# pdh930105/ARCQuant

Measured on AMD Instinct MI355X. Metric: ARC-NVFP4 GEMM TFLOP/s (M=4096, N=KQ=4096, KE=64), higher is better.
Workload: dtype f16

## Files before the change

arcquant_amd/agemm.py:

```python
from __future__ import annotations

import functools

import torch

from . import _lib
from ._lib import VARIANT_G16, VARIANT_G32, OUT_BF16, OUT_F32, ArcqError

_raw_stream = getattr(torch._C, "_cuda_getCurrentRawStream", None)


def _stream(t: torch.Tensor) -> int:
    if _raw_stream is not None:
        return _raw_stream(t.get_device())
    return torch.cuda.current_stream(t.device).cuda_stream


class _on:
    __slots__ = ("ctx",)

    def __init__(self, device):
        idx = device.index
        self.ctx = None if idx is None or idx == torch.cuda.current_device() else torch.cuda.device(device)

# ... 47 lines not shown
        return float(scale_host), scale, scale.data_ptr()
    return float(scale_host) * float(scale), None, None


_OUT_CODES = {torch.bfloat16: OUT_BF16, torch.float32: OUT_F32}


def _out(out, M, N, out_dtype, like, who):
    code = _OUT_CODES.get(out_dtype)
    if code is None:
        raise RuntimeError(f"agemm.{who}: out_dtype must be bfloat16 or float32")
    if out is None:
        return torch.empty((M, N), dtype=out_dtype, device=like.device), code
    _need(out, out_dtype, "out", 2)
    if out.shape != (M, N):
        raise RuntimeError(f"agemm.{who}: out has the wrong shape, expected ({M}, {N})")
    return out, code


def _same_device(who: str, A: torch.Tensor, *ts):
    idx = A.get_device()
    if idx < 0:
        raise RuntimeError(f"agemm.{who}: the operands must live on the GPU (there is no CPU path)")
    for t in ts:
        if t is not None and t.get_device() != idx:
            raise RuntimeError(f"agemm.{who}: every operand must live on the GPU of the first one ({A.device}), got {t.device}")


def _debug_set_tile_overlap_tail(mode: int) -> None:
    fn = _lib.lib().arcq_debug_set_tile_overlap_tail
    fn.restype, fn.argtypes = None, [_lib._i32]
    fn(int(mode))
    rw_route.cache_clear()


@functools.lru_cache(maxsize=None)
def variant_for_kq(KQ: int) -> int:
    return int(_lib.lib().arcq_variant_for_kq(int(KQ)))


@functools.lru_cache(maxsize=None)
def sf_buffer_bytes(rows: int, K: int) -> int:
    return int(_lib.lib().arcq_sf_alloc_bytes(int(rows), int(K)))


@functools.lru_cache(maxsize=None)
def _sf_used(rows: int, K: int) -> int:
    return int(_lib.lib().arcq_sf_used_bytes(int(rows), int(K)))


@functools.lru_cache(maxsize=None)
def _repacked_bytes(N: int, K: int):
    L = _lib.lib()
    return int(L.arcq_repacked_w_bytes(N, K)), int(L.arcq_repacked_sf_bytes(N, K))


def _need_repacked(RW, RSF, SFA, M, N, K, who, n_mult=1):
    _need(RW, torch.uint8, "RW", 1)
    _need(RSF, torch.uint8, "RSF", 1)
    if K % 64 or N % n_mult or (RW.numel(), RSF.numel()) != _repacked_bytes(N, K):
        raise RuntimeError(f"Value error in {who}: RW / RSF do not belong to a [{N}, {K}] weight" + (f", or N % {n_mult} != 0" if n_mult > 1 else ""))
    if SFA is not None and SFA.numel() < _sf_used(M, K):
        raise RuntimeError(f"Value error in {who}: SFA smaller than the swizzled layout of A")


def _quantize(fn_name: str, X: torch.Tensor, reorder_index: torch.Tensor, KE: int, variant):
# ... 475 lines not shown
```

arcquant_amd/csrc/arcq_internal.hpp:

```cpp
#pragma once
#include <hip/hip_runtime.h>
#include <stdint.h>
#include <stdlib.h>

#include "../../include/arcq.h"

namespace arcq {

int fail(int code, const char* fmt, ...) __attribute__((format(printf, 2, 3)));

inline int env_int(const char* name, int dflt) {
  const char* e = getenv(name);
  return e ? atoi(e) : dflt;
}

constexpr int kMaxDevices = 64;
struct LdsOptIn {
  int granted[kMaxDevices];
};
int ensure_dynamic_lds(const void* kernel, LdsOptIn& cache, int bytes, const char* who);

struct LdsBytes {
  int launch, optin;
  LdsBytes(int bytes) : launch(bytes), optin(bytes) {}
// ... 91 lines not shown
  const uint16_t* X;
  const uint16_t* Wn;
  float eps;
  const int16_t* idx;
  const uint32_t* in_slots;
  int n_in_slots;
  float* scale_out;
  const uint8_t* RW;
  const uint8_t* RSF;
  void* D;
  uint32_t* out_slots;
  const int16_t* act_scatter;
  int M, N, KQ, KE, variant;
  float alpha_host;
  const float* alpha_dev;
  const uint16_t* bias;
  const uint16_t* residual;
  int out_dtype;
};
int gemm_fused_supported(int kind, int64_t M, int64_t N, int64_t KQ, int64_t KE);
int gemm_fused(const FusedArgs& f, hipStream_t stream);
int64_t gemm_skinny_workspace_bytes(int64_t M, int64_t N, int64_t K);
int64_t gemm_tile_workspace_bytes(int64_t M, int64_t N, int64_t K);
int64_t gemm_tile_silu_slots(int64_t M, int64_t N, int64_t K);
int64_t gemm_decode_silu_slots(int64_t M, int64_t N, int64_t K);
int gemm_splitk_finish(const GemmArgs& a, int splitk, hipStream_t stream);
int gemm_skinny(const GemmArgs& a, hipStream_t stream);
int64_t gemm_decode_workspace_bytes(int64_t M, int64_t N, int64_t K);
int gemm_decode(const GemmArgs& a, hipStream_t stream);
int gemm_tile(const GemmArgs& a, hipStream_t stream);
int gemm_tile_repacked(const GemmArgs& a, hipStream_t stream);
int tile_overlap_tail_mode();
inline bool tile_overlap_tail_forced(int64_t M, int64_t N) { return tile_overlap_tail_mode() == 2 && M % 256 == 0 && N % 256 == 0; }
int gemm_regtile_cfg(int64_t M, int64_t N, int64_t K, int epilogue);
int gemm_regtile(const GemmArgs& a, int cfg, hipStream_t stream);
int gemm_regtile_fits(int64_t M, int64_t N, int64_t K, int b_layout);

struct KvWriteArgs {
  void* kv_data;
  void* kv_param;
  const int32_t *kv_indptr, *kv_indices, *last_page_offset;
  const void *k, *v, *k_param, *v_param;
  const int32_t* seqlen_indptr;
  int64_t ntok, B, L, layer, N, P;
  int format, dtype;
  bool quantize;
};
int kv_write(const KvWriteArgs& a, hipStream_t stream);
struct KvDecodeArgs {
  void* o;
  const void *q, *kv_data, *kv_param;
  const int32_t *kv_indptr, *kv_indices, *last_page_offset;
  int64_t B, Nq, L, layer, N, P, nnz;
  int format, dtype;
  void* workspace;
};
int kv_decode_splits(int64_t B, int64_t Nq, int64_t N, int64_t nnz, int64_t P);
int kv_decode(const KvDecodeArgs& a, hipStream_t stream);
struct KvStepArgs {
  const void *k, *v;
  int64_t q_stride, kv_stride;
  void* state;
};
int64_t kv_decode_chunks(int64_t Nq, int64_t N);
int kv_decode_step(const KvDecodeArgs& a, const KvStepArgs& st, hipStream_t stream);

// ... 13 lines not shown
```

arcquant_amd/csrc/gemm_tile.hip:

```cpp
#include <hip/hip_runtime.h>
#include <stdint.h>
#include <stdlib.h>

#include <type_traits>

#include "arcq_internal.hpp"
#include "gemm_common.hpp"
#include "gemm_tile_common.hpp"

namespace arcq {

#ifdef ARCQ_STREAM_STAMPS
#ifndef ARCQ_TILE_OT_UNIT
static unsigned long long* g_tile_stamps = nullptr;
#ifndef ARCQ_TILE_REPACKED_UNIT
extern "C" void arcq_debug_set_tile_stamps(void* p) { g_tile_stamps = reinterpret_cast<unsigned long long*>(p); }
#endif
#endif
#define ARCQ_TILE_STAMP(k)                                                                                     \
  do {                                                                                                         \
    if (p.stamps && tid == 0) {                                                                                \
      unsigned long long t0_, t1_;                                                                             \
      asm volatile("s_memtime %0\n\ts_memrealtime %1\n\ts_waitcnt lgkmcnt(0)" : "=s"(t0_), "=s"(t1_)::"memory"); \
      p.stamps[(size_t)blockIdx.x * (2 * kTileStamps) + 2 * (k)] = t0_;                                        \
      p.stamps[(size_t)blockIdx.x * (2 * kTileStamps) + 2 * (k) + 1] = t1_;                                    \
    }                                                                                                          \
  } while (0)
#else
#define ARCQ_TILE_STAMP(k) do { } while (0)
#endif

#ifndef ARCQ_TILE_WIDE_STORES
#define ARCQ_TILE_WIDE_STORES 1
#endif

#ifndef ARCQ_TILE_BARRIER_AT_STEP_END
#define ARCQ_TILE_BARRIER_AT_STEP_END 0
#endif
#ifndef ARCQ_TILE_ROT
#define ARCQ_TILE_ROT 1
#endif

#ifndef ARCQ_TILE_OT_UNIT
template <int BM, int BN, int WAVES_M, int WAVES_N, bool kMfma32, int kEpi, bool kStagger, bool kPipe, int kBLayout = kBRef>
__global__ __launch_bounds__(WAVES_M* WAVES_N * 64) void gemm_tile_kernel(TileParams p) {
  constexpr bool kOverlapTail = false;
  [[maybe_unused]] constexpr int kEpiOps = 0;
#else
template <int BM, int BN, int WAVES_M, int WAVES_N, int kEpi, int kBLayout, int kEpiOps>
__global__ __launch_bounds__(WAVES_M* WAVES_N * 64) void gemm_tile_ot_kernel(TileParams p) {
  static_assert(kEpiOps >= 0 && kEpiOps < (kEpi == kEpiSiluMul ? 2 : 4), "bit 0 bias, bit 1 residual (SiLU * up has no residual)");
  constexpr bool kMfma32 = false, kStagger = false, kPipe = true, kOverlapTail = true;
#endif
  constexpr int kThreads = WAVES_M * WAVES_N * 64;
  constexpr int WM = BM / WAVES_M, WN = BN / WAVES_N;
  constexpr int kT = kMfma32 ? 32 : 16;
  constexpr int TM = WM / kT, TN = WN / kT;
  using acc_t = typename std::conditional<kMfma32, f32x16, f32x4>::type;
  constexpr int A_UNITS = (BM * 2 + kThreads - 1) / kThreads, B_UNITS = (BN * 2 + kThreads - 1) / kThreads;
  constexpr bool A_PARTIAL = (BM * 2) % kThreads != 0, B_PARTIAL = (BN * 2) % kThreads != 0;
  static_assert(!A_PARTIAL || A_UNITS == 1, "a partial A pass is a single pass");
  static_assert(!B_PARTIAL || B_UNITS == 1, "a partial B pass is a single pass");
  constexpr int A_TILE = BM * kRowBytes, B_TILE = BN * kRowBytes;

  extern __shared__ __attribute__((aligned(16))) unsigned char smem[];
  unsigned char* const lds_a0 = smem;
  unsigned char* const lds_b0 = smem + A_TILE;
  unsigned char* const lds_a1 = smem + A_TILE + B_TILE;
  unsigned char* const lds_b1 = smem + 2 * A_TILE + B_TILE;

  const int ntiles = p.tiles_m * p.tiles_n;
  int bid = blockIdx.x, split = 0;
  if (p.splits > 1) {
    split = bid / ntiles;
    bid -= split * ntiles;
  }
  {
    const int q8 = ntiles >> 3, r8 = ntiles & 7, x = bid & 7, j = bid >> 3;
    bid = (x < r8 ? x * (q8 + 1) : r8 * (q8 + 1) + (x - r8) * q8) + j;
  }
  constexpr int kGroupM = 8;
  const int per_group = kGroupM * p.tiles_n;
  const int grp = bid / per_group;
  const int first_m = grp * kGroupM;
  const int gsz = min(p.tiles_m - first_m, kGroupM);
// ... 49 lines not shown
    if constexpr (kBLayout == kBRepacked) {
      const uint32_t rb = (uint32_t)((rc >> 4) - (n0 >> 4));
      b_q[u] = rb * (uint32_t)rw_tiles * 1024u + h * 256 + (rc & 15) * 16;
      b_sf[u] = rb * (uint32_t)rw_tiles * 128u + h * 64 + (rc & 15) * 4;
    } else {
      b_q[u] = (uint32_t)(rc - n0) * (uint32_t)half_k + h * 16;
      b_sf[u] = (uint32_t)(sf_atom_offset(rc, 0, atoms_k) - sf_atom_offset(n0, 0, atoms_k)) + h * 2;
    }
    b_live[u] = row < p.N ? kSfLive : 0u;
#pragma unroll
    for (int j = 0; j < 4; ++j) b_slot[u][j] = kMfma32 ? lds_slot32(r, h * 4 + j) : lds_slot(r, h * 4 + j);
  }
  const int fa_base = kMfma32 ? lds_slot32(wr * WM + (lane & 31), lane >> 5) : lds_slot(wr * WM + (lane & 15), lane >> 4);
  const int fb_base = kMfma32 ? lds_slot32(wc * WN + (lane & 31), lane >> 5) : lds_slot(wc * WN + (lane & 15), lane >> 4);
  acc_t acc[TM][TN];
  if constexpr (!kOverlapTail) {
#pragma unroll
    for (int i = 0; i < TM; ++i)
#pragma unroll
      for (int j = 0; j < TN; ++j)
#pragma unroll
        for (int r = 0; r < (kMfma32 ? 16 : 4); ++r) acc[i][j][r] = 0.f;
  }

  Staged sa[A_UNITS], sb[B_UNITS];
  auto load_step = [&](int atom) {
    atom = __builtin_amdgcn_readfirstlane(atom);
    const StageStep sa_step = stage_step(atom), sb_step = kBLayout == kBRepacked ? stage_step_rw(atom) : sa_step;
#pragma unroll
    for (int u = 0; u < A_UNITS; ++u) sa[u] = stage_load(a_src, a_q[u], a_sf[u], sa_step);
#pragma unroll
    for (int u = 0; u < B_UNITS; ++u) sb[u] = stage_load(b_src, b_q[u], b_sf[u], sb_step);
  };
  auto store_step = [&](unsigned char* la, unsigned char* lb) {
#pragma unroll
    for (int u = 0; u < A_UNITS; ++u)
      if (!A_PARTIAL || tid < BM * 2) stage_store(la, a_slot[u], sa[u], a_live[u]);
#pragma unroll
    for (int u = 0; u < B_UNITS; ++u)
      if (!B_PARTIAL || tid < BN * 2) stage_store(lb, b_slot[u], sb[u], b_live[u]);
  };
  auto mma_step = [&](const unsigned char* la, const unsigned char* lb) {
    if constexpr (kMfma32) {
#pragma unroll
      for (int ks = 0; ks < 4; ++ks) {
        Frag8 fa[TM], fb[TN];
#pragma unroll
        for (int i = 0; i < TM; ++i) fa[i].u = *reinterpret_cast<const uint4*>(la + (fa_base ^ (ks * 32)) + i * 32 * kRowBytes);
#pragma unroll
        for (int j = 0; j < TN; ++j) fb[j].u = *reinterpret_cast<const uint4*>(lb + (fb_base ^ (ks * 32)) + j * 32 * kRowBytes);
#pragma unroll
        for (int i = 0; i < TM; ++i)
#pragma unroll
          for (int j = 0; j < TN; ++j) acc[i][j] = __builtin_amdgcn_mfma_f32_32x32x16_f16(fb[j].v, fa[i].v, acc[i][j], 0, 0, 0);
      }
    } else {
#pragma unroll
      for (int ks = 0; ks < 2; ++ks) {
        Frag8 fa[TM], fb[TN];
#pragma unroll
        for (int i = 0; i < TM; ++i) fa[i].u = *reinterpret_cast<const uint4*>(la + (fa_base ^ (ks * 64)) + i * 16 * kRowBytes);
#pragma unroll
        for (int j = 0; j < TN; ++j) fb[j].u = *reinterpret_cast<const uint4*>(lb + (fb_base ^ (ks * 64)) + j * 16 * kRowBytes);
#pragma unroll
        for (int i = 0; i < TM; ++i)
#pragma unroll
          for (int j = 0; j < TN; ++j) acc[i][j] = __builtin_amdgcn_mfma_f32_16x16x32_f16(fb[j].v, fa[i].v, acc[i][j], 0, 0, 0);
      }
    }
  };
  const bool late = kStagger && wave >= 4;
  auto k_step = [&](int kt, unsigned char* ca, unsigned char* cb, unsigned char* na, unsigned char* nb) {
    Staged ta[A_UNITS], tb[B_UNITS];
#pragma unroll
    for (int u = 0; u < A_UNITS; ++u) ta[u] = sa[u];
#pragma unroll
    for (int u = 0; u < B_UNITS; ++u) tb[u] = sb[u];
    load_step(min(kt + 2 + (late ? 1 : 0), a_end - 1));
    __builtin_amdgcn_sched_barrier(0);
    mma_step(ca, cb);
    if (kStagger && late) __syncthreads();
    unsigned char* const wa = late ? ca : na;
    unsigned char* const wb = late ? cb : nb;
#pragma unroll
    for (int u = 0; u < A_UNITS; ++u)
      if (!A_PARTIAL || tid < BM * 2) stage_store(wa, a_slot[u], ta[u], a_live[u]);
#pragma unroll
    for (int u = 0; u < B_UNITS; ++u)
      if (!B_PARTIAL || tid < BN * 2) stage_store(wb, b_slot[u], tb[u], b_live[u]);
    if (!kStagger || !late) __syncthreads();
  };

  constexpr int kRot = ARCQ_TILE_ROT;
  constexpr bool kRotate = !ARCQ_TILE_BARRIER_AT_STEP_END && kPipe && !kMfma32 && TM == 8 && TN == 4 && WAVES_M * WAVES_N == 8 && !A_PARTIAL && !B_PARTIAL;
  auto rd_frag = [&](const unsigned char* tile, int base, int ks, int i) { Frag8 f; f.u = *reinterpret_cast<const uint4*>(tile + (base ^ (ks * 64)) + i * 16 * kRowBytes); return f; };
  [[maybe_unused]] Frag8 head_b[TN], head_a[2];
  auto k_step_pipe = [&](int kt, unsigned char* ca, unsigned char* cb, unsigned char* na, unsigned char* nb) {
    static_assert(kMfma32 || TM % 2 == 0, "pairs of A fragments");
    Staged ta[A_UNITS], tb[B_UNITS];
#pragma unroll
    for (int u = 0; u < A_UNITS; ++u) ta[u] = sa[u];
#pragma unroll
    for (int u = 0; u < B_UNITS; ++u) tb[u] = sb[u];
    load_step(min(kt + 2, a_end - 1));
    __builtin_amdgcn_sched_barrier(0);
    constexpr int kPieces = (A_UNITS + B_UNITS) * 4, kBlocks = kMfma32 ? 4 : TM;
    auto pieces = [&](int blk) {
#pragma unroll
      for (int c = blk; c < kPieces; c += kBlocks) {
        const int u = c >> 2, j = c & 3;
        if (u < A_UNITS) {
#ifdef ARCQ_EXPERIMENT_A_RAW
          if (!A_PARTIAL || tid < BM * 2) stage_piece_raw(na, a_slot[u < A_UNITS ? u : 0][j], ta[u < A_UNITS ? u : 0], a_live[u < A_UNITS ? u : 0], j);
#else
          if (!A_PARTIAL || tid < BM * 2) stage_piece(na, a_slot[u < A_UNITS ? u : 0][j], ta[u < A_UNITS ? u : 0], a_live[u < A_UNITS ? u : 0], j);
#endif
        } else {
          const int v = u - A_UNITS < B_UNITS ? u - A_UNITS : 0;
#ifdef ARCQ_EXPERIMENT_B_RAW
          if (!B_PARTIAL || tid < BN * 2) stage_piece_raw(nb, b_slot[v][j], tb[v], b_live[v], j);
#else
          if (!B_PARTIAL || tid < BN * 2) stage_piece(nb, b_slot[v][j], tb[v], b_live[v], j);
#endif
        }
      }
    };
    if constexpr (kMfma32) {
      Frag8 f32a[2][TM], f32b[2][TN];
      auto rd_set = [&](int buf, int ks) {
#pragma unroll
        for (int i = 0; i < TM; ++i) f32a[buf][i].u = *reinterpret_cast<const uint4*>(ca + (fa_base ^ (ks * 32)) + i * 32 * kRowBytes);
#pragma unroll
        for (int j = 0; j < TN; ++j) f32b[buf][j].u = *reinterpret_cast<const uint4*>(cb + (fb_base ^ (ks * 32)) + j * 32 * kRowBytes);
      };
      rd_set(0, 0);
#pragma unroll
      for (int ks = 0; ks < 4; ++ks) {
        if (ks + 1 < 4) rd_set((ks + 1) & 1, ks + 1);
        __builtin_amdgcn_sched_barrier(0);
#pragma unroll
        for (int i = 0; i < TM; ++i)
#pragma unroll
          for (int j = 0; j < TN; ++j)
            if constexpr (kMfma32)
              acc[i][j] = __builtin_amdgcn_mfma_f32_32x32x16_f16(f32b[ks & 1][j].v, f32a[ks & 1][i].v, acc[i][j], 0, 0, 0);
        pieces(ks);
        __builtin_amdgcn_sched_barrier(0);
      }
      __syncthreads();
      return;
    }
    auto rd_a = [&](int ks, int i) { return rd_frag(ca, fa_base, ks, i); };
    auto rd_b = [&](int ks, int j) { return rd_frag(cb, fb_base, ks, j); };
    if constexpr (kRotate) {
      constexpr int kQ = 2 * (TM / 2), kHalf = TM / 2, kLast = kQ - 1 - kRot, kNPre = kLast + 1;
      static_assert(kRot >= 1 && kLast >= kHalf, "the second K half's B fragments are read ahead of the barrier, a block before their use");
      auto read_by = [](int b) { const int extra = b - (kLast - kRot), h = b + 1 + (extra > 0 ? extra : 0); return h < kQ - 1 ? h : kQ - 1; };
      Frag8 fb1[TN], fq[kQ][2];
      fq[0][0] = head_a[0];
      fq[0][1] = head_a[1];
#pragma unroll
      for (int q = 0; q < kQ; ++q) {
        const int ks = q / kHalf, pr = q % kHalf;
        constexpr int kHeadReads = TN + 2;
        int n_pieces = 0, n_reads = 0;
        if (q <= kLast) {
#pragma unroll
          for (int r = (q ? read_by(q - 1) : 0) + 1; r <= read_by(q); ++r) {
            fq[r][0] = rd_a(r / kHalf, 2 * (r % kHalf));
            fq[r][1] = rd_a(r / kHalf, 2 * (r % kHalf) + 1);
          }
          if (q == kHalf - 1) {
#pragma unroll
            for (int j = 0; j < TN; ++j) fb1[j] = rd_b(1, j);
          }
        }
        __builtin_amdgcn_sched_barrier(0);
#pragma unroll
        for (int ii = 0; ii < 2; ++ii)
#pragma unroll
          for (int j = 0; j < TN; ++j)
            acc[2 * pr + ii][j] = __builtin_amdgcn_mfma_f32_16x16x32_f16((ks ? fb1[j] : head_b[j]).v, fq[q][ii].v, acc[2 * pr + ii][j], 0, 0, 0);
        if (q <= kLast) {
#pragma unroll
          for (int c = 0; c < kPieces; ++c)
            if (c * kNPre / kPieces == q) {
              const int u = c >> 2, j = c & 3;
              if (u < A_UNITS) {
                if (j == 0) asm volatile("" : "+v"(ta[u].sf));
                stage_piece(na, a_slot[u][j], ta[u], a_live[u], j);
              } else {
                if (j == 0) asm volatile("" : "+v"(tb[u - A_UNITS].sf));
                stage_piece(nb, b_slot[u - A_UNITS][j], tb[u - A_UNITS], b_live[u - A_UNITS], j);
              }
              ++n_pieces;
            }
        } else {
          const int i0 = q - kLast - 1;
// ... 29 lines not shown
      fq[q][0] = rd_a(q / kPairs, 2 * (q % kPairs));
      fq[q][1] = rd_a(q / kPairs, 2 * (q % kPairs) + 1);
    };
#pragma unroll
    for (int j = 0; j < TN; ++j) fb[0][j] = rd_b(0, j);
#pragma unroll
    for (int q = 0; q < kAhead; ++q) rd_pair(q);
#pragma unroll
    for (int q = 0; q < kSeq; ++q) {
      const int ks = q / kPairs, pr = q % kPairs;
      if (q + kAhead < kSeq) rd_pair(q + kAhead);
      if (ks == 0 && pr == kPairs - 1 - (kAhead - 1 < kPairs - 1 ? kAhead - 1 : kPairs - 1)) {
#pragma unroll
        for (int j = 0; j < TN; ++j) fb[1][j] = rd_b(1, j);
      }
      __builtin_amdgcn_sched_barrier(0);
#pragma unroll
      for (int ii = 0; ii < 2; ++ii)
#pragma unroll
        for (int j = 0; j < TN; ++j)
          if constexpr (!kMfma32)
            acc[2 * pr + ii][j] = __builtin_amdgcn_mfma_f32_16x16x32_f16(fb[ks][j].v, fq[q][ii].v, acc[2 * pr + ii][j], 0, 0, 0);
      pieces(q);
#pragma unroll
      for (int m8 = 0; m8 < (TM == 8 ? 2 * TN : 0); ++m8) {
        __builtin_amdgcn_sched_group_barrier(0x008, 1, 0);
        __builtin_amdgcn_sched_group_barrier(0x002, 2, 0);
      }
      __builtin_amdgcn_sched_barrier(0);
    }
    __syncthreads();
  };

  load_step(a_begin);
  Staged sa0[A_UNITS], sb0[B_UNITS];
#pragma unroll
  for (int u = 0; u < A_UNITS; ++u) sa0[u] = sa[u];
#pragma unroll
  for (int u = 0; u < B_UNITS; ++u) sb0[u] = sb[u];
  load_step(min(a_begin + 1, a_end - 1));
  __builtin_amdgcn_sched_barrier(0);
  if constexpr (kOverlapTail) {
#pragma unroll
    for (int i = 0; i < TM; ++i)
#pragma unroll
      for (int j = 0; j < TN; ++j) {
        acc[i][j] = acc_t{};
        asm volatile("" : "+v"(acc[i][j]));
      }
    __builtin_amdgcn_sched_barrier(0);
  }
#pragma unroll
  for (int u = 0; u < A_UNITS; ++u)
    if (!A_PARTIAL || tid < BM * 2) stage_store(lds_a0, a_slot[u], sa0[u], a_live[u]);
#pragma unroll
  for (int u = 0; u < B_UNITS; ++u)
    if (!B_PARTIAL || tid < BN * 2) stage_store(lds_b0, b_slot[u], sb0[u], b_live[u]);
  if (kStagger && late) {
    store_step(lds_a1, lds_b1);
    load_step(min(a_begin + 2, a_end - 1));
  }
  __syncthreads();
  if constexpr (kRotate) {
#pragma unroll
    for (int j = 0; j < TN; ++j) head_b[j] = rd_frag(lds_b0, fb_base, 0, j);
    head_a[0] = rd_frag(lds_a0, fa_base, 0, 0);
    head_a[1] = rd_frag(lds_a0, fa_base, 0, 1);
  }
  int kt = a_begin;
#ifndef ARCQ_EXPERIMENT_GENERAL_EPILOGUE
  float alpha_dev = 1.0f;
  if (p.alpha_dev) alpha_dev = *reinterpret_cast<const __attribute__((address_space(4))) float*>(reinterpret_cast<uintptr_t>(p.alpha_dev));
  asm volatile("" : "+s"(alpha_dev));
#endif
  if (WAVES_M * WAVES_N == 8 && wave >= 4) __builtin_amdgcn_s_setprio(1);
  ARCQ_TILE_STAMP(1);
  [[maybe_unused]] int tail_buf = 0;
  if constexpr (kOverlapTail) {
    static_assert(kRotate, "the final step is entered with head fragments");
    for (; kt + 2 < a_end; kt += 2) {
      k_step_pipe(kt, lds_a0, lds_b0, lds_a1, lds_b1);
      k_step_pipe(kt + 1, lds_a1, lds_b1, lds_a0, lds_b0);
    }
    if (kt + 1 < a_end) {
      k_step_pipe(kt, lds_a0, lds_b0, lds_a1, lds_b1);
      tail_buf = A_TILE + B_TILE;
    }
  } else if constexpr (kPipe) {
    for (; kt + 1 < a_end; kt += 2) {
      k_step_pipe(kt, lds_a0, lds_b0, lds_a1, lds_b1);
      k_step_pipe(kt + 1, lds_a1, lds_b1, lds_a0, lds_b0);
    }
    if (kt < a_end) k_step_pipe(kt, lds_a0, lds_b0, lds_a1, lds_b1);
  } else {
    for (; kt + 1 < a_end; kt += 2) {
      k_step(kt, lds_a0, lds_b0, lds_a1, lds_b1);
      k_step(kt + 1, lds_a1, lds_b1, lds_a0, lds_b0);
    }
    if (kt < a_end) k_step(kt, lds_a0, lds_b0, lds_a1, lds_b1);
  }
  if constexpr (!kOverlapTail) ARCQ_TILE_STAMP(2);

#ifdef ARCQ_EXPERIMENT_GENERAL_EPILOGUE
  const float alpha = p.alpha_host * (p.alpha_dev ? *p.alpha_dev : 1.0f);
#else
  const float alpha = p.alpha_host * alpha_dev;
#endif
  const bool vec_ok = (p.N & 3) == 0;
  uint32_t act_max = 0;
  [[maybe_unused]] auto interior_epilogue = [&](auto has_bias, auto has_res) __attribute__((always_inline)) {
    constexpr bool kBias = decltype(has_bias)::value, kRes = decltype(has_res)::value;
    constexpr bool kSilu = kEpi == kEpiSiluMul;
    constexpr uint32_t kElem = kSilu ? 1 : 2;
    unsigned char* const tile_d = reinterpret_cast<unsigned char*>(p.D) + ((size_t)m0 * p.N + n0) * kElem;
    const unsigned char* const tile_r = kRes ? reinterpret_cast<const unsigned char*>(p.residual) + ((size_t)m0 * p.N + n0) * 2 : nullptr;
    uint32_t t = tid;
    asm volatile("" : "+v"(t));
    const uint32_t lane_row = (t >> 6) / WAVES_N * WM + (t & 15), lane_col = (t >> 6) % WAVES_N * WN + 4 * ((t >> 4) & 3);
    uint32_t off = lane_row * (uint32_t)p.N + lane_col;
    const uint32_t row_step = 16u * (uint32_t)p.N;
    constexpr bool kWide = ARCQ_TILE_WIDE_STORES && !kSilu && TN % 2 == 0;
    typedef uint32_t u32x4_a8 __attribute__((ext_vector_type(4), aligned(8)));
    [[maybe_unused]] const uint32_t g4 = (t >> 4) & 3;
    [[maybe_unused]] uint32_t off_w = off - 4 * g4 + ((g4 & 1) ? 16 + 4 * (g4 - 1) : 4 * g4);
    [[maybe_unused]] uint2 held = make_uint2(0, 0);
    constexpr bool kPackedBias = kOverlapTail && kBias && kRes;
// ... 252 lines not shown
        for (int j = 0; j < TN; ++j) {
          store4(mb + i * 16, nb + j * 16, acc[i][j][0], acc[i][j][1], acc[i][j][2], acc[i][j][3], true, bias_v[j], res_cur[j]);
          if (i == 0 && j == 0) ARCQ_TILE_STAMP(3);
        }
#pragma unroll
        for (int j = 0; j < TN; ++j) res_cur[j] = res_nxt[j];
      }
    } else {
#pragma unroll
      for (int i = 0; i < TM; ++i)
#pragma unroll
        for (int j = 0; j < TN; ++j) {
          store4(mb + i * 16, nb + j * 16, acc[i][j][0], acc[i][j][1], acc[i][j][2], acc[i][j][3], false, make_uint2(0, 0), make_uint2(0, 0));
          if (i == 0 && j == 0) ARCQ_TILE_STAMP(3);
        }
    }
  }
  ARCQ_TILE_STAMP(4);
  if (kEpi == kEpiSiluMul) {
    __shared__ uint32_t wave_max[WAVES_M * WAVES_N];
#pragma unroll
    for (int sh = 32; sh > 0; sh >>= 1) act_max = max(act_max, (uint32_t)__shfl_down((int)act_max, sh, 64));
    if (lane == 0) wave_max[wave] = act_max;
    __syncthreads();
    if (tid == 0) {
      uint32_t m = 0;
#pragma unroll
      for (int w = 0; w < WAVES_M * WAVES_N; ++w) m = max(m, wave_max[w]);
      p.slots[blockIdx.x] = m;
    }
  }
}

#ifdef ARCQ_TILE_OT_UNIT
static int g_tile_overlap_tail = 1;
int tile_overlap_tail_mode() { return g_tile_overlap_tail; }
extern "C" void arcq_debug_set_tile_overlap_tail(int mode) { g_tile_overlap_tail = mode < 0 ? 0 : mode > 2 ? 2 : mode; }

template <int kEpi, int kBLayout, int kEpiOps>
static int launch_ot(const TileParams& p, dim3 grid, hipStream_t stream) {
  return launch_kernel<gemm_tile_ot_kernel<256, 256, 2, 4, kEpi, kBLayout, kEpiOps>>(grid, dim3(512), 2 * (256 + 256) * kRowBytes, stream,
                                                                                   "arcq_gemm_nvfp4 (tile, overlapped tail)", p);
}
template <int kEpi, int kBLayout>
static int launch_ot_ops(const TileParams& p, dim3 grid, hipStream_t stream) {
  const int ops = (p.bias ? 1 : 0) | (p.residual ? 2 : 0);
  if constexpr (kEpi == kEpiSiluMul) {
    return ops & 1 ? launch_ot<kEpi, kBLayout, 1>(p, grid, stream) : launch_ot<kEpi, kBLayout, 0>(p, grid, stream);
  } else {
    switch (ops) {
      case 1: return launch_ot<kEpi, kBLayout, 1>(p, grid, stream);
      case 2: return launch_ot<kEpi, kBLayout, 2>(p, grid, stream);
      case 3: return launch_ot<kEpi, kBLayout, 3>(p, grid, stream);
      default: return launch_ot<kEpi, kBLayout, 0>(p, grid, stream);
    }
  }
}
int launch_tile_overlap_tail(const TileParams& p, int epi, int b_layout, dim3 grid, hipStream_t stream) {
  if (epi == kEpiSiluMul) return b_layout == kBRepacked ? launch_ot_ops<kEpiSiluMul, kBRepacked>(p, grid, stream) : launch_ot_ops<kEpiSiluMul, kBRef>(p, grid, stream);
  return b_layout == kBRepacked ? launch_ot_ops<kEpiPlain, kBRepacked>(p, grid, stream) : launch_ot_ops<kEpiPlain, kBRef>(p, grid, stream);
}
#else

struct TileCfg { int id, bm, bn, waves; };
static constexpr TileCfg kTileCfgs[] = {{1, 128, 128, 4}, {2, 256, 256, 4}, {3, 256, 256, 8}, {4, 128, 256, 4}, {5, 256, 256, 8}, {6, 128, 128, 4},
                                        {7, 64, 256, 4}, {8, 32, 256, 4}, {9, 128, 128, 4}, {10, 128, 256, 8}, {11, 256, 128, 8}, {12, 128, 128, 8},
                                        {13, 64, 256, 8}, {14, 64, 128, 8}, {15, 64, 64, 4}, {16, 64, 128, 4}, {17, 128, 64, 4}};
// ... 38 lines not shown
static int launch_tile(const GemmArgs& a, hipStream_t stream, bool allow_split = false) {
  TileParams p;
  copy_gemm_fields(p, a);
  p.B = a.B; p.SFB = a.SFB;
  p.tiles_m = (a.M + BM - 1) / BM;
  p.tiles_n = (a.N + BN - 1) / BN;
  p.splits = 1; p.atoms_per_split = a.K / 64; p.partial = nullptr;
  p.epi = a.epilogue; p.slots = a.absmax_slots;
#ifdef ARCQ_STREAM_STAMPS
  p.stamps = g_tile_stamps;
#endif
  if (allow_split && a.epilogue == kEpiPlain) {
    tile_split(a.M, a.N, a.K, BM, BN, &p.splits, &p.atoms_per_split);
    if (p.splits > 1) {
      const int64_t need = (int64_t)p.splits * a.M * a.N * (int64_t)sizeof(float);
      if (!a.workspace || a.workspace_bytes < need)
        return fail(ARCQ_ERR_WORKSPACE, "arcq_gemm_nvfp4: split-K needs %lld B of workspace, got %lld", (long long)need,
                    (long long)a.workspace_bytes);
      p.partial = reinterpret_cast<float*>(a.workspace);
    }
  }
  if (((int64_t)a.K + 255) / 256 * 256 * 128 > 0xffffffffll)
    return fail(ARCQ_ERR_SHAPE, "arcq_gemm_nvfp4 (tile): K = %lld: a tile's rows of an operand exceed 32-bit offsets", (long long)a.K);
  const int lds = 2 * (BM + BN) * kRowBytes;
  const dim3 grid((unsigned)(p.tiles_m * p.tiles_n * p.splits)), block(WAVES_M * WAVES_N * 64);
  const char* who = "arcq_gemm_nvfp4 (tile)";
  constexpr bool kCanStagger = WAVES_M * WAVES_N == 8 && BM == 256 && BN == 256;
  const bool pipe = tile_pipe(), stagger = !pipe && kCanStagger && tile_stagger();
  int rc;
  bool overlap_tail = false;
  if constexpr (BM == 256 && BN == 256 && WAVES_M * WAVES_N == 8 && !kMfma32 && !ARCQ_TILE_BARRIER_AT_STEP_END)
    overlap_tail = pipe && (kEpi == kEpiSiluMul ? tile_overlap_tail_mode() == 2 : tile_overlap_tail_mode() != 0) && a.M % BM == 0 && a.N % BN == 0 && p.splits <= 1 && a.out_dtype == ARCQ_OUT_BF16 &&
                   (int64_t)BM * a.N < (1ll << 31) && ((reinterpret_cast<uintptr_t>(a.bias) | reinterpret_cast<uintptr_t>(a.residual)) & 7) == 0;
  if (overlap_tail) rc = launch_tile_overlap_tail(p, kEpi, kBLayout, grid, stream);
  else if (!pipe && !stagger) rc = launch_kernel<gemm_tile_kernel<BM, BN, WAVES_M, WAVES_N, kMfma32, kEpi, false, false, kBLayout>>(grid, block, lds, stream, who, p);
  else if (pipe) rc = launch_kernel<gemm_tile_kernel<BM, BN, WAVES_M, WAVES_N, kMfma32, kEpi, false, true, kBLayout>>(grid, block, lds, stream, who, p);
  else rc = launch_kernel<gemm_tile_kernel<BM, BN, WAVES_M, WAVES_N, kMfma32, kEpi, kCanStagger, false, kBLayout>>(grid, block, lds, stream, who, p);
  if (rc != ARCQ_OK) return rc;
  if (p.splits > 1) return gemm_splitk_finish(a, p.splits, stream);
  return ARCQ_OK;
}

static int tile_choice(int64_t M, int64_t N, int64_t K) {
  const int64_t t256 = ((M + 255) / 256) * ((N + 255) / 256);
  if (t256 >= 192) return 3;
  if (M <= 32) return 8;
  if (M <= 64) return 7;
  const int64_t t10 = ((M + 127) / 128) * ((N + 255) / 256);
  if (t10 <= 64 || t10 == 128 || (t10 > 224 && t10 <= 256) || (K >= 8192 && t10 >= 96 && t10 <= 256)) return 10;
  return 1;
}

static int effective_cfg(int64_t M, int64_t N, int64_t K, bool* may_split) {
  int id = tile_cfg_override();
  if (id == 0) id = tile_overlap_tail_forced(M, N) ? 3 : tile_choice(M, N, K);
  id = tile_cfg(id).id;
  *may_split = !(id >= 2 && id <= 6) && id != 9;
  return id;
}

#ifndef ARCQ_TILE_REPACKED_UNIT
int64_t gemm_tile_silu_slots(int64_t M, int64_t N, int64_t K) {
  bool sp;
  const TileCfg& c = tile_cfg(effective_cfg(M, N, K, &sp));
  return ((M + c.bm - 1) / c.bm) * ((N + c.bn - 1) / c.bn);
}

// ... 46 lines not shown
```

arcquant_amd/csrc/gemm_tile_common.hpp:

```cpp
#pragma once
#include <hip/hip_runtime.h>
#include <stdint.h>

#include "arcq_internal.hpp"
#include "gemm_common.hpp"

namespace arcq {

struct TileParams {
  const uint8_t* A;
  const uint8_t* B;
  const uint8_t* SFA;
  const uint8_t* SFB;
  void* D;
  const float* alpha_dev;
  const uint16_t* bias;
  const uint16_t* residual;
  int M, N, K;
  float alpha_host;
  int out_dtype;
  int tiles_m, tiles_n;
  int splits, atoms_per_split;
  float* partial;
  int epi;
  unsigned int* slots;
#ifdef ARCQ_STREAM_STAMPS
  unsigned long long* stamps;
#endif
};
constexpr int kTileStamps = 5;
int launch_tile_overlap_tail(const TileParams& p, int epi, int b_layout, dim3 grid, hipStream_t stream);

constexpr int kBK = 64;
constexpr int kRowBytes = kBK * 2;

__device__ __forceinline__ int lds_slot(int r, int ks) { return r * kRowBytes + ((ks ^ (r & 7)) << 4); }
__device__ __forceinline__ int lds_slot32(int r, int ks) { return r * kRowBytes + ((ks ^ ((r >> 1) & 7)) << 4); }

struct Staged {
  uint4 q;
  uint32_t sf;
};

typedef uint32_t u32x4 __attribute__((ext_vector_type(4)));
typedef __amdgpu_buffer_rsrc_t buf_rsrc;

__device__ __forceinline__ buf_rsrc stage_rsrc(const uint8_t* base, uint32_t bytes) {
  return __builtin_amdgcn_make_buffer_rsrc(const_cast<uint8_t*>(base), 0, (int)bytes, 0x00020000);
}

struct StageSrc {
  buf_rsrc q, sf;
};
struct StageStep {
  uint32_t q, sf;
};
__device__ __forceinline__ StageStep stage_step(int atom) { return {(uint32_t)atom * 32u, (uint32_t)atom * 512u}; }
__device__ __forceinline__ StageStep stage_step_rw(int atom) {
  return {(uint32_t)atom * 512u, (uint32_t)((atom >> 2) * 256 + (atom & 1) * 128 + ((atom >> 1) & 1) * 2)};
}
__device__ __forceinline__ Staged stage_load(const StageSrc& src, uint32_t q_lane, uint32_t sf_lane, StageStep step) {
  Staged s;
  const u32x4 q = __builtin_amdgcn_raw_buffer_load_b128(src.q, (int)q_lane, (int)step.q, 0);
  s.q = make_uint4(q.x, q.y, q.z, q.w);
  s.sf = (uint16_t)__builtin_amdgcn_raw_buffer_load_b16(src.sf, (int)sf_lane, (int)step.sf, 0);
  return s;
}

constexpr uint32_t kSfLive = 0x3f803f80u;
__device__ __forceinline__ f16x2 sf_pair_both(uint32_t sf16, uint32_t live_mask) {
  const uint32_t w = ((sf16 << 7) | (sf16 << 15)) & live_mask;
  f16x2 r;
  __builtin_memcpy(&r, &w, 4);
  return r;
}
template <int kHalf>
__device__ __forceinline__ f16x2 sf_splat(f16x2 s) { return __builtin_shufflevector(s, s, kHalf, kHalf); }

__device__ __forceinline__ void stage_piece(unsigned char* tile, int slot, const Staged& s, uint32_t live_mask, int j) {
  const uint32_t w = j == 0 ? s.q.x : j == 1 ? s.q.y : j == 2 ? s.q.z : s.q.w;
  const f16x2 sf = sf_pair_both(s.sf, live_mask);
  const Frag8 f = dequant8(w, j < 2 ? sf_splat<0>(sf) : sf_splat<1>(sf));
  *reinterpret_cast<uint4*>(tile + slot) = f.u;
}

#if defined(ARCQ_EXPERIMENT_A_RAW) || defined(ARCQ_EXPERIMENT_B_RAW)
__device__ __forceinline__ void stage_piece_raw(unsigned char* tile, int slot, const Staged& s, uint32_t live_mask, int j) {
  const uint32_t w = (j == 0 ? s.q.x : j == 1 ? s.q.y : j == 2 ? s.q.z : s.q.w) & (live_mask ? 0x3bff3bffu : 0u);
  *reinterpret_cast<uint4*>(tile + slot) = make_uint4(w, w, w, w);
}
#endif

__device__ __forceinline__ void stage_store(unsigned char* tile, const int (&slot)[4], const Staged& s, uint32_t live_mask) {
  const f16x2 sf = sf_pair_both(s.sf, live_mask);
  const f16x2 s0 = sf_splat<0>(sf), s1 = sf_splat<1>(sf);
  Frag8 f0 = dequant8(s.q.x, s0), f1 = dequant8(s.q.y, s0), f2 = dequant8(s.q.z, s1), f3 = dequant8(s.q.w, s1);
  *reinterpret_cast<uint4*>(tile + slot[0]) = f0.u;
  *reinterpret_cast<uint4*>(tile + slot[1]) = f1.u;
  *reinterpret_cast<uint4*>(tile + slot[2]) = f2.u;
// ... 6 lines not shown
```

Baseline: 1474.

## Add paired-load tile kernel variant issuing two k-steps of global loads together

Adds a sibling compilation unit of the overlap-tail tile GEMM kernel that fetches the staged A/B quantized data and scale factors for two consecutive k-steps in one batch every other step. The loads are interleaved across the MFMA phases, and the odd step consumes the prefetched second buffer. The aim is to cut how often global loads are issued and to group them so more memory latency is hidden. It costs extra staging registers, which may lower occupancy or cause spills. It is enabled by default for the plain epilogue on the overlap-tail path.

Measured after the change: 1496 (median of 6 runs). 1.5% higher.

```diff
diff --git a/arcquant_amd/agemm.py b/arcquant_amd/agemm.py
--- a/arcquant_amd/agemm.py
+++ b/arcquant_amd/agemm.py
@@ -103,6 +103,12 @@
     fn.restype, fn.argtypes = None, [_lib._i32]
     fn(int(mode))
     rw_route.cache_clear()
+
+
+def _debug_set_tile_pair_loads(on: int) -> None:
+    fn = _lib.lib().arcq_debug_set_tile_pair_loads
+    fn.restype, fn.argtypes = None, [_lib._i32]
+    fn(int(on))
 
 
 @functools.lru_cache(maxsize=None)
diff --git a/arcquant_amd/csrc/arcq_internal.hpp b/arcquant_amd/csrc/arcq_internal.hpp
--- a/arcquant_amd/csrc/arcq_internal.hpp
+++ b/arcquant_amd/csrc/arcq_internal.hpp
@@ -147,6 +147,7 @@
 int gemm_tile_repacked(const GemmArgs& a, hipStream_t stream);
 int tile_overlap_tail_mode();
 inline bool tile_overlap_tail_forced(int64_t M, int64_t N) { return tile_overlap_tail_mode() == 2 && M % 256 == 0 && N % 256 == 0; }
+int tile_pair_loads_mode();
 int gemm_regtile_cfg(int64_t M, int64_t N, int64_t K, int epilogue);
 int gemm_regtile(const GemmArgs& a, int cfg, hipStream_t stream);
 int gemm_regtile_fits(int64_t M, int64_t N, int64_t K, int b_layout);
diff --git a/arcquant_amd/csrc/gemm_tile.hip b/arcquant_amd/csrc/gemm_tile.hip
--- a/arcquant_amd/csrc/gemm_tile.hip
+++ b/arcquant_amd/csrc/gemm_tile.hip
@@ -8,10 +8,14 @@
 #include "gemm_common.hpp"
 #include "gemm_tile_common.hpp"
 
+#if defined(ARCQ_TILE_OT_UNIT) || defined(ARCQ_TILE_PL_UNIT)
+#define ARCQ_TILE_SIBLING_UNIT
+#endif
+
 namespace arcq {
 
 #ifdef ARCQ_STREAM_STAMPS
-#ifndef ARCQ_TILE_OT_UNIT
+#ifndef ARCQ_TILE_SIBLING_UNIT
 static unsigned long long* g_tile_stamps = nullptr;
 #ifndef ARCQ_TILE_REPACKED_UNIT
 extern "C" void arcq_debug_set_tile_stamps(void* p) { g_tile_stamps = reinterpret_cast<unsigned long long*>(p); }
@@ -41,16 +45,21 @@
 #define ARCQ_TILE_ROT 1
 #endif
 
-#ifndef ARCQ_TILE_OT_UNIT
+#if defined(ARCQ_TILE_PL_UNIT)
+template <int BM, int BN, int WAVES_M, int WAVES_N, int kEpi, int kBLayout, int kEpiOps>
+__global__ __launch_bounds__(WAVES_M* WAVES_N * 64) void gemm_tile_pl_kernel(TileParams p) {
+  static_assert(kEpi == kEpiPlain && kEpiOps >= 0 && kEpiOps < 4, "bit 0 bias, bit 1 residual (SiLU * up keeps gemm_tile_ot_kernel)");
+  constexpr bool kMfma32 = false, kStagger = false, kPipe = true, kOverlapTail = true, kPairLoads = true;
+#elif !defined(ARCQ_TILE_OT_UNIT)
 template <int BM, int BN, int WAVES_M, int WAVES_N, bool kMfma32, int kEpi, bool kStagger, bool kPipe, int kBLayout = kBRef>
 __global__ __launch_bounds__(WAVES_M* WAVES_N * 64) void gemm_tile_kernel(TileParams p) {
-  constexpr bool kOverlapTail = false;
+  constexpr bool kOverlapTail = false, kPairLoads = false;
   [[maybe_unused]] constexpr int kEpiOps = 0;
 #else
 template <int BM, int BN, int WAVES_M, int WAVES_N, int kEpi, int kBLayout, int kEpiOps>
 __global__ __launch_bounds__(WAVES_M* WAVES_N * 64) void gemm_tile_ot_kernel(TileParams p) {
   static_assert(kEpiOps >= 0 && kEpiOps < (kEpi == kEpiSiluMul ? 2 : 4), "bit 0 bias, bit 1 residual (SiLU * up has no residual)");
-  constexpr bool kMfma32 = false, kStagger = false, kPipe = true, kOverlapTail = true;
+  constexpr bool kMfma32 = false, kStagger = false, kPipe = true, kOverlapTail = true, kPairLoads = false;
 #endif
   constexpr int kThreads = WAVES_M * WAVES_N * 64;
   constexpr int WM = BM / WAVES_M, WN = BN / WAVES_N;
@@ -166,6 +175,51 @@
 #pragma unroll
     for (int u = 0; u < B_UNITS; ++u) sb[u] = stage_load(b_src, b_q[u], b_sf[u], sb_step);
   };
+#ifdef ARCQ_TILE_PL_UNIT
+  Staged sa2[A_UNITS], sb2[B_UNITS];
+  auto load_pair = [&](int atom0, int atom1, Staged (&a0)[A_UNITS], Staged (&b0)[B_UNITS], Staged (&a1)[A_UNITS], Staged (&b1)[B_UNITS], auto parts) {
+    constexpr int kParts = decltype(parts)::value;
+    atom0 = __builtin_amdgcn_readfirstlane(atom0);
+    atom1 = __builtin_amdgcn_readfirstlane(atom1);
+    const StageStep a_s0 = stage_step(atom0), a_s1 = stage_step(atom1);
+    const StageStep b_s0 = kBLayout == kBRepacked ? stage_step_rw(atom0) : a_s0, b_s1 = kBLayout == kBRepacked ? stage_step_rw(atom1) : a_s1;
+    __builtin_amdgcn_sched_barrier(0);
+    if constexpr ((kParts & 1) != 0) {
+#pragma unroll
+      for (int u = 0; u < A_UNITS; ++u) {
+        a0[u].q = stage_load_q(a_src, a_q[u], a_s0);
+        __builtin_amdgcn_sched_barrier(0);
+        a1[u].q = stage_load_q(a_src, a_q[u], a_s1);
+        __builtin_amdgcn_sched_barrier(0);
+      }
+    }
+    if constexpr ((kParts & 2) != 0) {
+#pragma unroll
+      for (int u = 0; u < B_UNITS; ++u) {
+        b0[u].q = stage_load_q(b_src, b_q[u], b_s0);
+        __builtin_amdgcn_sched_barrier(0);
+        b1[u].q = stage_load_q(b_src, b_q[u], b_s1);
+        __builtin_amdgcn_sched_barrier(0);
+      }
+    }
+    if constexpr ((kParts & 4) != 0) {
+#pragma unroll
+      for (int u = 0; u < A_UNITS; ++u) {
+        a0[u].sf = stage_load_sf(a_src, a_sf[u], a_s0);
+        a1[u].sf = stage_load_sf(a_src, a_sf[u], a_s1);
+      }
+#pragma unroll
+      for (int u = 0; u < B_UNITS; ++u) {
+        b0[u].sf = stage_load_sf(b_src, b_sf[u], b_s0);
+        b1[u].sf = stage_load_sf(b_src, b_sf[u], b_s1);
+      }
+    }
+  };
+  using kPairA = std::integral_constant<int, 1>;
+  using kPairB = std::integral_constant<int, 2>;
+  using kPairSf = std::integral_constant<int, 4>;
+  using kPairAll = std::integral_constant<int, 7>;
+#endif
   auto store_step = [&](unsigned char* la, unsigned char* lb) {
 #pragma unroll
     for (int u = 0; u < A_UNITS; ++u)
@@ -229,14 +283,29 @@
   constexpr bool kRotate = !ARCQ_TILE_BARRIER_AT_STEP_END && kPipe && !kMfma32 && TM == 8 && TN == 4 && WAVES_M * WAVES_N == 8 && !A_PARTIAL && !B_PARTIAL;
   auto rd_frag = [&](const unsigned char* tile, int base, int ks, int i) { Frag8 f; f.u = *reinterpret_cast<const uint4*>(tile + (base ^ (ks * 64)) + i * 16 * kRowBytes); return f; };
   [[maybe_unused]] Frag8 head_b[TN], head_a[2];
-  auto k_step_pipe = [&](int kt, unsigned char* ca, unsigned char* cb, unsigned char* na, unsigned char* nb) {
+  using kStepOne = std::integral_constant<int, 0>;
+  using kStepPair = std::integral_constant<int, 1>;
+  using kStepOdd = std::integral_constant<int, 2>;
+  using kStepNone = std::integral_constant<int, 3>;
+  auto k_step_pipe = [&](int kt, unsigned char* ca, unsigned char* cb, unsigned char* na, unsigned char* nb, auto step_kind) {
     static_assert(kMfma32 || TM % 2 == 0, "pairs of A fragments");
+    constexpr int kKind = decltype(step_kind)::value;
+    static_assert(kKind == 0 || kPairLoads, "the paired-load sibling's steps");
     Staged ta[A_UNITS], tb[B_UNITS];
 #pragma unroll
     for (int u = 0; u < A_UNITS; ++u) ta[u] = sa[u];
 #pragma unroll
     for (int u = 0; u < B_UNITS; ++u) tb[u] = sb[u];
-    load_step(min(kt + 2, a_end - 1));
+    if constexpr (kKind == kStepOne::value) load_step(min(kt + 2, a_end - 1));
+#ifdef ARCQ_TILE_PL_UNIT
+    if constexpr (kKind == kStepOdd::value) {
+#pragma unroll
+      for (int u = 0; u < A_UNITS; ++u) ta[u] = sa2[u];
+#pragma unroll
+      for (int u = 0; u < B_UNITS; ++u) tb[u] = sb2[u];
+    }
+    if constexpr (kKind == kStepPair::value) load_pair(min(kt + 2, a_end - 1), min(kt + 3, a_end - 1), sa2, sb2, sa, sb, kPairA{});
+#endif
     __builtin_amdgcn_sched_barrier(0);
     constexpr int kPieces = (A_UNITS + B_UNITS) * 4, kBlocks = kMfma32 ? 4 : TM;
     auto pieces = [&](int blk) {
@@ -298,6 +367,13 @@
         const int ks = q / kHalf, pr = q % kHalf;
         constexpr int kHeadReads = TN + 2;
         int n_pieces = 0, n_reads = 0;
+#ifdef ARCQ_TILE_PL_UNIT
+        if constexpr (kKind == kStepPair::value) {
+          if (q == 2) load_pair(min(kt + 2, a_end - 1), min(kt + 3, a_end - 1), sa2, sb2, sa, sb, kPairB{});
+          if (q == 4) load_pair(min(kt + 2, a_end - 1), min(kt + 3, a_end - 1), sa2, sb2, sa, sb, kPairSf{});
+          if (q == 2 || q == 4) __builtin_amdgcn_sched_barrier(0);
+        }
+#endif
         if (q <= kLast) {
 #pragma unroll
           for (int r = (q ? read_by(q - 1) : 0) + 1; r <= read_by(q); ++r) {
@@ -393,6 +469,10 @@
     __syncthreads();
   };
 
+#ifdef ARCQ_TILE_PL_UNIT
+  Staged sa0[A_UNITS], sb0[B_UNITS];
+  load_pair(a_begin, min(a_begin + 1, a_end - 1), sa0, sb0, sa, sb, kPairAll{});
+#else
   load_step(a_begin);
   Staged sa0[A_UNITS], sb0[B_UNITS];
 #pragma unroll
@@ -400,6 +480,7 @@
 #pragma unroll
   for (int u = 0; u < B_UNITS; ++u) sb0[u] = sb[u];
   load_step(min(a_begin + 1, a_end - 1));
+#endif
   __builtin_amdgcn_sched_barrier(0);
   if constexpr (kOverlapTail) {
 #pragma unroll
@@ -439,20 +520,23 @@
   [[maybe_unused]] int tail_buf = 0;
   if constexpr (kOverlapTail) {
     static_assert(kRotate, "the final step is entered with head fragments");
+    using Even = std::conditional_t<kPairLoads, kStepPair, kStepOne>;
+    using Odd = std::conditional_t<kPairLoads, kStepOdd, kStepOne>;
+    using Last = std::conditional_t<kPairLoads, kStepNone, kStepOne>;
     for (; kt + 2 < a_end; kt += 2) {
-      k_step_pipe(kt, lds_a0, lds_b0, lds_a1, lds_b1);
-      k_step_pipe(kt + 1, lds_a1, lds_b1, lds_a0, lds_b0);
+      k_step_pipe(kt, lds_a0, lds_b0, lds_a1, lds_b1, Even{});
+      k_step_pipe(kt + 1, lds_a1, lds_b1, lds_a0, lds_b0, Odd{});
     }
     if (kt + 1 < a_end) {
-      k_step_pipe(kt, lds_a0, lds_b0, lds_a1, lds_b1);
+      k_step_pipe(kt, lds_a0, lds_b0, lds_a1, lds_b1, Last{});
       tail_buf = A_TILE + B_TILE;
     }
   } else if constexpr (kPipe) {
     for (; kt + 1 < a_end; kt += 2) {
-      k_step_pipe(kt, lds_a0, lds_b0, lds_a1, lds_b1);
-      k_step_pipe(kt + 1, lds_a1, lds_b1, lds_a0, lds_b0);
-    }
-    if (kt < a_end) k_step_pipe(kt, lds_a0, lds_b0, lds_a1, lds_b1);
+      k_step_pipe(kt, lds_a0, lds_b0, lds_a1, lds_b1, kStepOne{});
+      k_step_pipe(kt + 1, lds_a1, lds_b1, lds_a0, lds_b0, kStepOne{});
+    }
+    if (kt < a_end) k_step_pipe(kt, lds_a0, lds_b0, lds_a1, lds_b1, kStepOne{});
   } else {
     for (; kt + 1 < a_end; kt += 2) {
       k_step(kt, lds_a0, lds_b0, lds_a1, lds_b1);
@@ -771,7 +855,29 @@
   }
 }
 
-#ifdef ARCQ_TILE_OT_UNIT
+#if defined(ARCQ_TILE_PL_UNIT)
+static int g_tile_pair_loads = 1;
+int tile_pair_loads_mode() { return g_tile_pair_loads; }
+extern "C" void arcq_debug_set_tile_pair_loads(int on) { g_tile_pair_loads = on != 0; }
+
+template <int kBLayout, int kEpiOps>
+static int launch_pl(const TileParams& p, dim3 grid, hipStream_t stream) {
+  return launch_kernel<gemm_tile_pl_kernel<256, 256, 2, 4, kEpiPlain, kBLayout, kEpiOps>>(grid, dim3(512), 2 * (256 + 256) * kRowBytes, stream,
+                                                                                        "arcq_gemm_nvfp4 (tile, paired loads)", p);
+}
+template <int kBLayout>
+static int launch_pl_ops(const TileParams& p, dim3 grid, hipStream_t stream) {
+  switch ((p.bias ? 1 : 0) | (p.residual ? 2 : 0)) {
+    case 1: return launch_pl<kBLayout, 1>(p, grid, stream);
+    case 2: return launch_pl<kBLayout, 2>(p, grid, stream);
+    case 3: return launch_pl<kBLayout, 3>(p, grid, stream);
+    default: return launch_pl<kBLayout, 0>(p, grid, stream);
+  }
+}
+int launch_tile_pair_loads(const TileParams& p, int b_layout, dim3 grid, hipStream_t stream) {
+  return b_layout == kBRepacked ? launch_pl_ops<kBRepacked>(p, grid, stream) : launch_pl_ops<kBRef>(p, grid, stream);
+}
+#elif defined(ARCQ_TILE_OT_UNIT)
 static int g_tile_overlap_tail = 1;
 int tile_overlap_tail_mode() { return g_tile_overlap_tail; }
 extern "C" void arcq_debug_set_tile_overlap_tail(int mode) { g_tile_overlap_tail = mode < 0 ? 0 : mode > 2 ? 2 : mode; }
@@ -876,7 +982,8 @@
   if constexpr (BM == 256 && BN == 256 && WAVES_M * WAVES_N == 8 && !kMfma32 && !ARCQ_TILE_BARRIER_AT_STEP_END)
     overlap_tail = pipe && (kEpi == kEpiSiluMul ? tile_overlap_tail_mode() == 2 : tile_overlap_tail_mode() != 0) && a.M % BM == 0 && a.N % BN == 0 && p.splits <= 1 && a.out_dtype == ARCQ_OUT_BF16 &&
                    (int64_t)BM * a.N < (1ll << 31) && ((reinterpret_cast<uintptr_t>(a.bias) | reinterpret_cast<uintptr_t>(a.residual)) & 7) == 0;
-  if (overlap_tail) rc = launch_tile_overlap_tail(p, kEpi, kBLayout, grid, stream);
+  if (overlap_tail && kEpi == kEpiPlain && tile_pair_loads_mode() != 0) rc = launch_tile_pair_loads(p, kBLayout, grid, stream);
+  else if (overlap_tail) rc = launch_tile_overlap_tail(p, kEpi, kBLayout, grid, stream);
   else if (!pipe && !stagger) rc = launch_kernel<gemm_tile_kernel<BM, BN, WAVES_M, WAVES_N, kMfma32, kEpi, false, false, kBLayout>>(grid, block, lds, stream, who, p);
   else if (pipe) rc = launch_kernel<gemm_tile_kernel<BM, BN, WAVES_M, WAVES_N, kMfma32, kEpi, false, true, kBLayout>>(grid, block, lds, stream, who, p);
   else rc = launch_kernel<gemm_tile_kernel<BM, BN, WAVES_M, WAVES_N, kMfma32, kEpi, kCanStagger, false, kBLayout>>(grid, block, lds, stream, who, p);
diff --git a/arcquant_amd/csrc/gemm_tile_common.hpp b/arcquant_amd/csrc/gemm_tile_common.hpp
--- a/arcquant_amd/csrc/gemm_tile_common.hpp
+++ b/arcquant_amd/csrc/gemm_tile_common.hpp
@@ -30,6 +30,7 @@
 };
 constexpr int kTileStamps = 5;
 int launch_tile_overlap_tail(const TileParams& p, int epi, int b_layout, dim3 grid, hipStream_t stream);
+int launch_tile_pair_loads(const TileParams& p, int b_layout, dim3 grid, hipStream_t stream);
 
 constexpr int kBK = 64;
 constexpr int kRowBytes = kBK * 2;
@@ -65,6 +66,13 @@
   s.q = make_uint4(q.x, q.y, q.z, q.w);
   s.sf = (uint16_t)__builtin_amdgcn_raw_buffer_load_b16(src.sf, (int)sf_lane, (int)step.sf, 0);
   return s;
+}
+__device__ __forceinline__ uint4 stage_load_q(const StageSrc& src, uint32_t q_lane, StageStep step) {
+  const u32x4 q = __builtin_amdgcn_raw_buffer_load_b128(src.q, (int)q_lane, (int)step.q, 0);
+  return make_uint4(q.x, q.y, q.z, q.w);
+}
+__device__ __forceinline__ uint32_t stage_load_sf(const StageSrc& src, uint32_t sf_lane, StageStep step) {
+  return (uint16_t)__builtin_amdgcn_raw_buffer_load_b16(src.sf, (int)sf_lane, (int)step.sf, 0);
 }
 
 constexpr uint32_t kSfLive = 0x3f803f80u;
diff --git a/arcquant_amd/csrc/gemm_tile_pl.hip b/arcquant_amd/csrc/gemm_tile_pl.hip
--- /dev/null
+++ b/arcquant_amd/csrc/gemm_tile_pl.hip
@@ -0,0 +1,2 @@
+#define ARCQ_TILE_PL_UNIT
+#include "gemm_tile.hip"
```
